# NthPortal/reservoir

Hardware: AMD Instinct MI355X
Metric: elements sampled/sec (Gelem/s) + % HBM roofline, 1B Long keys k=1024, 1/2/4/8 GPU (higher is better)
Workload: dtype int64

## Files before the change

reservoir_amd/csrc/rsv_device.h:

```cpp
#pragma once
#include <hip/hip_runtime.h>
#include <stdint.h>

namespace rsv {

struct u32x4 {
    uint32_t x, y, z, w;
};

constexpr uint32_t kPhiloxM0 = 0xD2511F53u;
constexpr uint32_t kPhiloxM1 = 0xCD9E8D57u;
constexpr uint32_t kPhiloxW0 = 0x9E3779B9u;
constexpr uint32_t kPhiloxW1 = 0xBB67AE85u;
constexpr uint32_t kDomainLevel1 = 0x80000000u;

__device__ __forceinline__ uint32_t xor3_key(uint32_t a, uint32_t b, uint32_t key) {
    return __builtin_amdgcn_bitop3_b32(a, b, key, 0x96);
}

__device__ __forceinline__ u32x4 philox4x32_10(uint32_t c0, uint32_t c1, uint32_t c2, uint32_t c3,
                                               uint32_t k0, uint32_t k1) {
#pragma unroll
    for (int r = 0; r < 10; ++r) {
        const uint64_t p0 = (uint64_t)kPhiloxM0 * c0;
        const uint64_t p1 = (uint64_t)kPhiloxM1 * c2;
        const uint32_t n0 = xor3_key((uint32_t)(p1 >> 32), c1, k0 + (uint32_t)r * kPhiloxW0);
        const uint32_t n2 = xor3_key((uint32_t)(p0 >> 32), c3, k1 + (uint32_t)r * kPhiloxW1);
        c0 = n0;
        c1 = (uint32_t)p1;
        c2 = n2;
        c3 = (uint32_t)p0;
    }
    return {c0, c1, c2, c3};
}

__device__ __forceinline__ u32x4 philox4x32_10_uniform_hi(uint32_t c0, uint32_t c1, uint32_t c2, uint32_t c3,
                                                          uint32_t k0, uint32_t k1, uint64_t add0 = 0) {
    const uint64_t p1u = (uint64_t)kPhiloxM1 * c2;
    const uint32_t n0u = (uint32_t)(p1u >> 32) ^ c1 ^ k0;
    const uint64_t p0 = (uint64_t)kPhiloxM0 * c0 + add0;
    uint32_t d2 = (uint32_t)(p0 >> 32) ^ (c3 ^ k1);
    const uint32_t d1u = (uint32_t)p1u;
    uint32_t d3 = (uint32_t)p0;
    const uint64_t q0u = (uint64_t)kPhiloxM0 * n0u;
    const uint64_t q1 = (uint64_t)kPhiloxM1 * d2;
    uint32_t c0v = (uint32_t)(q1 >> 32) ^ (d1u ^ (k0 + kPhiloxW0));
    uint32_t c2v = d3 ^ ((uint32_t)(q0u >> 32) ^ (k1 + kPhiloxW1));
    uint32_t c1v = (uint32_t)q1;
    uint32_t c3v = (uint32_t)q0u;
    {
        const uint64_t p0r = (uint64_t)kPhiloxM0 * c0v;
        const uint64_t p1r = (uint64_t)kPhiloxM1 * c2v;
        const uint32_t n0 = xor3_key((uint32_t)(p1r >> 32), c1v, k0 + 2u * kPhiloxW0);
        const uint32_t n2 = (uint32_t)(p0r >> 32) ^ (c3v ^ (k1 + 2u * kPhiloxW1));
        c0v = n0;
        c1v = (uint32_t)p1r;
        c2v = n2;
        c3v = (uint32_t)p0r;
    }
#pragma unroll
    for (int r = 3; r < 10; ++r) {
        const uint64_t p0r = (uint64_t)kPhiloxM0 * c0v;
        const uint64_t p1r = (uint64_t)kPhiloxM1 * c2v;
        const uint32_t n0 = xor3_key((uint32_t)(p1r >> 32), c1v, k0 + (uint32_t)r * kPhiloxW0);
        const uint32_t n2 = xor3_key((uint32_t)(p0r >> 32), c3v, k1 + (uint32_t)r * kPhiloxW1);
        c0v = n0;
        c1v = (uint32_t)p1r;
        c2v = n2;
        c3v = (uint32_t)p0r;
    }
    return {c0v, c1v, c2v, c3v};
}

__device__ __forceinline__ void philox4x32_10_uniform_hi_x2(uint32_t c0, uint32_t c1, uint32_t c2, uint32_t c3,
                                                            uint32_t k0, uint32_t k1, u32x4& a, u32x4& b) {
    const uint64_t p1u = (uint64_t)kPhiloxM1 * c2;
    const uint32_t n0u = (uint32_t)(p1u >> 32) ^ c1 ^ k0;
    const uint64_t pa = (uint64_t)kPhiloxM0 * c0;
    const uint64_t pb = (uint64_t)kPhiloxM0 * c0 + (uint64_t)kPhiloxM0 * 64u;
    const uint32_t da2 = xor3_key((uint32_t)(pa >> 32), c3, k1), db2 = xor3_key((uint32_t)(pb >> 32), c3, k1);
    const uint32_t d1u = (uint32_t)p1u;
    const uint32_t da3 = (uint32_t)pa, db3 = (uint32_t)pb;
    const uint64_t q0u = (uint64_t)kPhiloxM0 * n0u;
    const uint64_t qa = (uint64_t)kPhiloxM1 * da2, qb = (uint64_t)kPhiloxM1 * db2;
    uint32_t a0 = (uint32_t)(qa >> 32) ^ (d1u ^ (k0 + kPhiloxW0)), b0 = (uint32_t)(qb >> 32) ^ (d1u ^ (k0 + kPhiloxW0));
    uint32_t a2 = da3 ^ ((uint32_t)(q0u >> 32) ^ (k1 + kPhiloxW1)), b2 = db3 ^ ((uint32_t)(q0u >> 32) ^ (k1 + kPhiloxW1));
    uint32_t a1 = (uint32_t)qa, b1 = (uint32_t)qb;
    uint32_t a3 = (uint32_t)q0u, b3 = (uint32_t)q0u;
#pragma unroll
    for (int r = 2; r < 10; ++r) {
        const uint64_t pa0 = (uint64_t)kPhiloxM0 * a0, pb0 = (uint64_t)kPhiloxM0 * b0;
        const uint64_t pa1 = (uint64_t)kPhiloxM1 * a2, pb1 = (uint64_t)kPhiloxM1 * b2;
        const uint32_t na0 = xor3_key((uint32_t)(pa1 >> 32), a1, k0 + (uint32_t)r * kPhiloxW0);
        const uint32_t nb0 = xor3_key((uint32_t)(pb1 >> 32), b1, k0 + (uint32_t)r * kPhiloxW0);
        const uint32_t na2 = xor3_key((uint32_t)(pa0 >> 32), a3, k1 + (uint32_t)r * kPhiloxW1);
        const uint32_t nb2 = xor3_key((uint32_t)(pb0 >> 32), b3, k1 + (uint32_t)r * kPhiloxW1);
        a0 = na0;
        b0 = nb0;
        a1 = (uint32_t)pa1;
        b1 = (uint32_t)pb1;
        a2 = na2;
        b2 = nb2;
        a3 = (uint32_t)pa0;
        b3 = (uint32_t)pb0;
    }
    a = {a0, a1, a2, a3};
    b = {b0, b1, b2, b3};
}

constexpr uint32_t kPhiloxM0Inv = 0x991A7CDBu;
static_assert((uint32_t)(kPhiloxM0 * kPhiloxM0Inv) == 1u, "M0 inverse");

__device__ __forceinline__ void philox4x32_10_uniform_hi_x2_at(uint32_t gl, uint32_t m0v, uint64_t offa,
                                                               uint32_t c1, uint32_t c2, uint32_t c3,
                                                               uint32_t k0, uint32_t k1, u32x4& a, u32x4& b,
                                                               uint32_t& lo_a) {
    const uint64_t p1u = (uint64_t)kPhiloxM1 * c2;
    const uint32_t n0u = (uint32_t)(p1u >> 32) ^ c1 ^ k0;
    const uint64_t pa = (uint64_t)m0v * gl + offa;
    const uint64_t pb = (uint64_t)m0v * gl + (offa + (uint64_t)kPhiloxM0 * 64u);
    lo_a = (uint32_t)pa;
    const uint32_t c3k = c3 ^ k1;
    const uint32_t da2 = (uint32_t)(pa >> 32) ^ c3k, db2 = (uint32_t)(pb >> 32) ^ c3k;
    const uint32_t d1u = (uint32_t)p1u;
    const uint32_t da3 = (uint32_t)pa, db3 = (uint32_t)pb;
    const uint64_t q0u = (uint64_t)kPhiloxM0 * n0u;
    const uint64_t qa = (uint64_t)kPhiloxM1 * da2, qb = (uint64_t)kPhiloxM1 * db2;
    uint32_t a0 = (uint32_t)(qa >> 32) ^ (d1u ^ (k0 + kPhiloxW0)), b0 = (uint32_t)(qb >> 32) ^ (d1u ^ (k0 + kPhiloxW0));
    uint32_t a2 = da3 ^ ((uint32_t)(q0u >> 32) ^ (k1 + kPhiloxW1)), b2 = db3 ^ ((uint32_t)(q0u >> 32) ^ (k1 + kPhiloxW1));
    uint32_t a1 = (uint32_t)qa, b1 = (uint32_t)qb;
    uint32_t a3 = (uint32_t)q0u, b3 = (uint32_t)q0u;
    {
        const uint64_t pa0 = (uint64_t)kPhiloxM0 * a0, pb0 = (uint64_t)kPhiloxM0 * b0;
        const uint64_t pa1 = (uint64_t)kPhiloxM1 * a2, pb1 = (uint64_t)kPhiloxM1 * b2;
        const uint32_t na0 = xor3_key((uint32_t)(pa1 >> 32), a1, k0 + 2u * kPhiloxW0);
        const uint32_t nb0 = xor3_key((uint32_t)(pb1 >> 32), b1, k0 + 2u * kPhiloxW0);
        const uint32_t s3 = (uint32_t)q0u ^ (k1 + 2u * kPhiloxW1);
        const uint32_t na2 = (uint32_t)(pa0 >> 32) ^ s3, nb2 = (uint32_t)(pb0 >> 32) ^ s3;
        a0 = na0;
        b0 = nb0;
        a1 = (uint32_t)pa1;
        b1 = (uint32_t)pb1;
        a2 = na2;
        b2 = nb2;
        a3 = (uint32_t)pa0;
        b3 = (uint32_t)pb0;
    }
#pragma unroll
    for (int r = 3; r < 10; ++r) {
        const uint64_t pa0 = (uint64_t)kPhiloxM0 * a0, pb0 = (uint64_t)kPhiloxM0 * b0;
        const uint64_t pa1 = (uint64_t)kPhiloxM1 * a2, pb1 = (uint64_t)kPhiloxM1 * b2;
        const uint32_t na0 = xor3_key((uint32_t)(pa1 >> 32), a1, k0 + (uint32_t)r * kPhiloxW0);
        const uint32_t nb0 = xor3_key((uint32_t)(pb1 >> 32), b1, k0 + (uint32_t)r * kPhiloxW0);
        const uint32_t na2 = xor3_key((uint32_t)(pa0 >> 32), a3, k1 + (uint32_t)r * kPhiloxW1);
        const uint32_t nb2 = xor3_key((uint32_t)(pb0 >> 32), b3, k1 + (uint32_t)r * kPhiloxW1);
        a0 = na0;
        b0 = nb0;
        a1 = (uint32_t)pa1;
        b1 = (uint32_t)pb1;
        a2 = na2;
        b2 = nb2;
        a3 = (uint32_t)pa0;
        b3 = (uint32_t)pb0;
    }
    a = {a0, a1, a2, a3};
    b = {b0, b1, b2, b3};
}

struct DrawKey {
    uint32_t k0, k1;
    uint32_t s0, s1;
};

__device__ __forceinline__ u32x4 level0(const DrawKey& dk, uint64_t g0) {
    return philox4x32_10((uint32_t)g0, (uint32_t)(g0 >> 32), dk.s0, dk.s1, dk.k0, dk.k1);
}

__device__ __forceinline__ uint32_t word_of(const u32x4& w, uint32_t q) {
    return q == 0 ? w.x : q == 1 ? w.y : q == 2 ? w.z : w.w;
}

__device__ __forceinline__ uint32_t level0_byte(const u32x4& w, uint32_t e) {
    const uint32_t u = ((w.x >> e) & 0x10001u) | (((w.y >> e) & 0x10001u) << 2) |
                       (((w.z >> e) & 0x10001u) << 4) | (((w.w >> e) & 0x10001u) << 6);
    return (u & 0x55u) | ((u >> 15) & 0xAAu);
}

__device__ __forceinline__ uint64_t exact_j(const DrawKey& dk, uint64_t i, uint32_t b) {
    const uint64_t g1 = i >> 1;
    const u32x4 w =
        philox4x32_10((uint32_t)g1, (uint32_t)(g1 >> 32) | kDomainLevel1, dk.s0, dk.s1, dk.k0, dk.k1);
    const uint64_t L = (i & 1) ? (((uint64_t)w.z << 32) | w.w) : (((uint64_t)w.x << 32) | w.y);
    const uint64_t U = ((uint64_t)b << 56) | (L >> 8);
    return __umul64hi(U, i + 1);
}

__device__ __forceinline__ uint32_t planes_or(const u32x4& w) {
    const uint32_t x = w.x | w.y | w.z | w.w;
    return x | __builtin_amdgcn_alignbit(x, x, 16);
}

__device__ __forceinline__ uint32_t zero_byte_mask16(const u32x4& w) { return ~planes_or(w) & 0xFFFFu; }

__device__ __forceinline__ bool any_zero_byte(const u32x4& w) { return planes_or(w) != 0xFFFFFFFFu; }

__device__ __forceinline__ uint32_t lt_mask16(const u32x4& w, uint32_t T) {
    if (T >= 256u) return 0xFFFFu;
    uint32_t lt = 0, eq = 0xFFFFu;
#pragma unroll
    for (int p = 7; p >= 0; --p) {
        const uint32_t plane = (word_of(w, (uint32_t)p >> 1) >> (16 * (p & 1))) & 0xFFFFu;
        const uint32_t tm = 0u - ((T >> p) & 1u);
        lt |= eq & ~plane & tm;
        eq &= ~(plane ^ tm);
    }
    return lt & 0xFFFFu;
}

__host__ __device__ __forceinline__ uint64_t bswap64(uint64_t v) { return __builtin_bswap64(v); }

__host__ __device__ __forceinline__ int64_t byteswap64(int64_t v) {
    uint64_t hc = (uint64_t)v * 0x9e3779b97f4a7c15ULL;
    hc = bswap64(hc);
    return (int64_t)(hc * 0x9e3779b97f4a7c15ULL);
}

__host__ __device__ __forceinline__ int64_t scramble(int64_t r0, int64_t r1, int64_t hashed) {
    return byteswap64(r1 ^ byteswap64(r0 ^ hashed));
}

enum HashKind : int { kHashIdentity = 1, kHashJavaLong = 2, kHashJavaInt = 3, kHashPrecomputed = 4, kHashUuid = 5 };

__host__ __device__ __forceinline__ int64_t uuid_hash_code(uint64_t msb, uint64_t lsb) {
    const uint64_t hilo = msb ^ lsb;
    return (int64_t)(int32_t)((uint32_t)(hilo >> 32) ^ (uint32_t)hilo);
}

enum WideSrc : int { kWideSrcHashes = 0, kWideSrcUuid = 1 };

template <typename KeyT, int HASH>
__host__ __device__ __forceinline__ int64_t hash_of(KeyT key) {
    if constexpr (HASH == kHashJavaLong) {
        const uint64_t v = (uint64_t)(int64_t)key;
        return (int64_t)(int32_t)(uint32_t)(v ^ (v >> 32));
    } else if constexpr (HASH == kHashJavaInt) {
        return (int64_t)(int32_t)key;
    } else {
        return (int64_t)key;
    }
}

__device__ __forceinline__ uint32_t xor_lane32(uint32_t v, int s) {
    switch (s) {
    case 1: return (uint32_t)__builtin_amdgcn_mov_dpp((int)v, 0xB1, 0xF, 0xF, false);
    case 2: return (uint32_t)__builtin_amdgcn_mov_dpp((int)v, 0x4E, 0xF, 0xF, false);
    case 4: {
        const uint32_t up = (uint32_t)__builtin_amdgcn_mov_dpp((int)v, 0x104, 0xF, 0xF, false);
        const uint32_t dn = (uint32_t)__builtin_amdgcn_mov_dpp((int)v, 0x114, 0xF, 0xF, false);
        return (threadIdx.x & 4) ? dn : up;
    }
    case 8: return (uint32_t)__builtin_amdgcn_mov_dpp((int)v, 0x128, 0xF, 0xF, false);
    case 16: {
        const auto r = __builtin_amdgcn_permlane16_swap(v, v, false, false);
        return (threadIdx.x & 16) ? r[0] : r[1];
    }
    case 32: {
        const auto r = __builtin_amdgcn_permlane32_swap(v, v, false, false);
        return (threadIdx.x & 32) ? r[0] : r[1];
    }
    default: return (uint32_t)__shfl_xor((int)v, s);
    }
}

template <typename T>
__device__ __forceinline__ T xor_any(T v, int s) {
    if constexpr (sizeof(T) == 8) {
        const uint64_t x = (uint64_t)v;
        const uint32_t lo = xor_lane32((uint32_t)x, s), hi = xor_lane32((uint32_t)(x >> 32), s);
        return (T)(((uint64_t)hi << 32) | lo);
    } else {
        return (T)xor_lane32((uint32_t)v, s);
    }
}

__device__ __forceinline__ unsigned long long lanemask_lt64() {
    const uint32_t lane = threadIdx.x & 63;
    return lane ? (~0ull >> (64 - lane)) : 0ull;
}

__device__ __forceinline__ void publish_flag(uint32_t* flag, uint32_t gen) {
    asm volatile("s_waitcnt vmcnt(0)" ::: "memory");
    __syncthreads();
    if (threadIdx.x == 0) {
        __threadfence_system();
        __hip_atomic_store(flag, gen, __ATOMIC_RELEASE, __HIP_MEMORY_SCOPE_SYSTEM);
    }
}

}
```

reservoir_amd/csrc/rsv_elements.hip:

```cpp
#include <algorithm>

#include "rsv_device.h"
#include "rsv_internal.h"
#include "rsv_scan.h"

namespace rsv {

namespace {

constexpr int kBlock = 256;

constexpr int kK1Unroll = 2;

constexpr unsigned kK1Grid = 256 * 20;

constexpr int kK1Win = 12;
struct K1Lds {
    uint64_t q[kBlock / 64][k1q_cap<kK1Win>()];
    uint64_t cq[kBlock / 64][kQueue];
};

__device__ __forceinline__ bool k1_fast(uint64_t lo, uint64_t hi) {
    return (lo >> 33) == ((hi - 1) >> 33) && hi <= (1ull << 40);
}

struct K1Sched {
    uint32_t W1, A, B;
};

__global__ __launch_bounds__(kBlock) void k1_last_writer(DrawKey dk, uint32_t k, uint64_t lo,
                                                         uint64_t hi, uint64_t g_begin,
                                                         uint64_t n_groups,
                                                         unsigned long long* __restrict__ win, K1Sched sch) {
    __shared__ K1Lds L;
    const int w = threadIdx.x >> 6;
    if (k1_fast(lo, hi))
        k1_body_q<kK1Win, true>(dk, k, lo, hi, g_begin, n_groups, win, L.q[w], L.cq[w], sch.W1, sch.A, sch.B);
    else
        k1_body_q<kK1Win, false>(dk, k, lo, hi, g_begin, n_groups, win, L.q[w], L.cq[w], sch.W1, sch.A, sch.B);
}

template <typename Take, typename Empty, typename Keep>
__device__ __forceinline__ void slot_rule(int64_t j, unsigned long long wi, int64_t base, int64_t n, int fresh,
                                          Take&& take, Empty&& empty, Keep&& keep) {
    if (wi) take((int64_t)wi - base, (int64_t)wi, true);
    else if (j >= base && j < base + n) take(j - base, j, false);
    else if (fresh) empty((int64_t)-1);
    else keep();
}

template <typename KeyT, int R, bool kAgentWin>
__device__ __forceinline__ void resolve_registers_first(const KeyT* __restrict__ keys, int64_t base, int64_t n,
                                                        uint32_t k, unsigned long long* __restrict__ win,
                                                        KeyT* __restrict__ slot_key, int64_t* __restrict__ slot_idx,
                                                        int fresh, int64_t m, KeyT* dst, uint32_t* flag, uint32_t gen) {
    unsigned long long wi[R];
    KeyT v[R];
#pragma unroll
    for (int r = 0; r < R; ++r) {
        const uint32_t j = threadIdx.x + r * kBlock;
        if (j >= k) wi[r] = 0ull;
        else if (kAgentWin) wi[r] = __hip_atomic_load(&win[j], __ATOMIC_RELAXED, __HIP_MEMORY_SCOPE_AGENT);
        else wi[r] = win[j];
    }
#pragma unroll
    for (int r = 0; r < R; ++r) {
        const int64_t j = threadIdx.x + r * kBlock;
        if (j >= k) continue;
        KeyT x;
        slot_rule(
            j, wi[r], base, n, fresh, [&](int64_t off, int64_t, bool) { x = keys[off]; }, [&](int64_t) { x = 0; },
            [&] { x = slot_key[j]; });
        v[r] = x;
    }
#pragma unroll
    for (int r = 0; r < R; ++r) {
        const int64_t j = threadIdx.x + r * kBlock;
        if (j >= k) continue;
        const KeyT x = v[r];
        slot_rule(
            j, wi[r], base, n, fresh,
            [=](int64_t, int64_t idx, bool winner) {
                slot_key[j] = x;
                slot_idx[j] = idx;
                if (winner) win[j] = 0;
            },
            [=](int64_t idx) {
                slot_key[j] = 0;
                slot_idx[j] = idx;
            },
            [] {});
        if (j < m) dst[j] = x;
    }
    publish_flag(flag, gen);
}

constexpr uint32_t kK1FusedMaxK = 8 * kBlock;

template <typename KeyT>
__global__ __launch_bounds__(kBlock) void k1_resolve_publish(DrawKey dk, uint32_t k, uint64_t lo, uint64_t hi,
                                                             uint64_t g_begin, uint64_t n_groups,
                                                             unsigned long long* __restrict__ win,
                                                             uint32_t* ticket, const KeyT* __restrict__ keys,
                                                             int64_t base, int64_t n, KeyT* __restrict__ slot_key,
                                                             int64_t* __restrict__ slot_idx, int fresh, int64_t m,
                                                             KeyT* dst, uint32_t* flag, uint32_t gen, K1Sched sch) {
    __shared__ K1Lds L;
    __shared__ uint32_t last;
    const int w = threadIdx.x >> 6;
    if (k1_fast(lo, hi))
        k1_body_q<kK1Win, true>(dk, k, lo, hi, g_begin, n_groups, win, L.q[w], L.cq[w], sch.W1, sch.A, sch.B);
    else
        k1_body_q<kK1Win, false>(dk, k, lo, hi, g_begin, n_groups, win, L.q[w], L.cq[w], sch.W1, sch.A, sch.B);
    asm volatile("s_waitcnt vmcnt(0)" ::: "memory");
    __syncthreads();
    if (threadIdx.x == 0) {
        const uint32_t prev = __hip_atomic_fetch_add(ticket, 1u, __ATOMIC_RELAXED, __HIP_MEMORY_SCOPE_AGENT);
        last = prev == gridDim.x - 1;
        if (last) __hip_atomic_store(ticket, 0u, __ATOMIC_RELAXED, __HIP_MEMORY_SCOPE_AGENT);
    }
    __syncthreads();
    if (!last) return;
    __builtin_amdgcn_fence(__ATOMIC_ACQUIRE, "agent");
    resolve_registers_first<KeyT, kK1FusedMaxK / kBlock, true>(keys, base, n, k, win, slot_key, slot_idx, fresh, m, dst,
                                                               flag, gen);
}

template <typename KeyT, bool kPublish>
__global__ __launch_bounds__(kPublish ? 1024 : kBlock) void resolve_kernel(const KeyT* __restrict__ keys, int64_t base,
                                                                         int64_t n, uint32_t k,
                                                                         unsigned long long* __restrict__ win,
                                                                         KeyT* __restrict__ slot_key,
                                                                         int64_t* __restrict__ slot_idx, int fresh,
                                                                         int64_t m, KeyT* dst, uint32_t* flag,
                                                                         uint32_t gen) {
    const uint32_t stride = gridDim.x * blockDim.x;
    for (uint32_t j = blockIdx.x * blockDim.x + threadIdx.x; j < k; j += stride) {
        KeyT v = 0;
        slot_rule(
            j, win[j], base, n, fresh,
            [&](int64_t off, int64_t idx, bool winner) {
                slot_key[j] = v = keys[off];
                if (kPublish || slot_idx) slot_idx[j] = idx;
                if (winner) win[j] = 0;
            },
            [=](int64_t idx) {
                slot_key[j] = 0;
                if (kPublish || slot_idx) slot_idx[j] = idx;
            },
            [&] {
                if (kPublish) v = slot_key[j];
            });
        if (kPublish && (int64_t)j < m) dst[j] = v;
    }
    if (kPublish) publish_flag(flag, gen);
}

template <typename KeyT, int R>
__global__ __launch_bounds__(kBlock) void resolve_publish_small_kernel(const KeyT* __restrict__ keys, int64_t base,
                                                                       int64_t n, uint32_t k,
                                                                       unsigned long long* __restrict__ win,
                                                                       KeyT* __restrict__ slot_key,
                                                                       int64_t* __restrict__ slot_idx, int fresh,
                                                                       int64_t m, KeyT* dst, uint32_t* flag, uint32_t gen) {
    resolve_registers_first<KeyT, R, false>(keys, base, n, k, win, slot_key, slot_idx, fresh, m, dst, flag, gen);
}

__global__ __launch_bounds__(kBlock) void replay_kernel(const int64_t* __restrict__ ev_pos,
                                                        const int32_t* __restrict__ ev_slot,
                                                        int64_t n_events, uint32_t k,
                                                        unsigned long long* __restrict__ win) {
    const int64_t e = (int64_t)blockIdx.x * blockDim.x + threadIdx.x;
    if (e >= n_events) return;
    const int32_t s = ev_slot[e];
    const int64_t p = ev_pos[e];
    if (s >= 0 && (uint32_t)s < k && p >= 2) atomicMax(&win[s], (unsigned long long)(p - 1));
}

__global__ __launch_bounds__(kBlock) void export_draws_kernel(DrawKey dk, uint64_t i0, int64_t n,
                                                              uint64_t* __restrict__ out) {
    const int64_t t = (int64_t)blockIdx.x * blockDim.x + threadIdx.x;
    if (t >= n) return;
    const uint64_t i = i0 + (uint64_t)t;
    const u32x4 w = level0(dk, i >> 4);
    out[t] = exact_j(dk, i, level0_byte(w, (uint32_t)(i & 15)));
}

template <typename KeyT>
struct StridedParts {
    using Key = KeyT;
    const int64_t* idx;
    const KeyT* key;
    int64_t part_len;
    __device__ int64_t index(int32_t p, uint32_t j) const { return idx[(int64_t)p * part_len + j]; }
    __device__ void take(int32_t p, uint32_t j, KeyT* slot_key) const { slot_key[j] = key[(int64_t)p * part_len + j]; }
};

template <typename KeyT>
struct PackedRows {
    using Key = KeyT;
    const int64_t* rows;
    int64_t stride;
    uint32_t k;
    __device__ int64_t index(int32_t p, uint32_t j) const { return rows[(int64_t)p * stride + j]; }
    __device__ void take(int32_t p, uint32_t j, KeyT* slot_key) const {
        slot_key[j] = (KeyT)rows[(int64_t)p * stride + k + j];
    }
};

struct StridedWideParts {
    using Key = uint32_t;
    const int64_t* idx;
    const uint32_t* key;
    int64_t part_len;
    uint32_t words;
    __device__ int64_t index(int32_t p, uint32_t j) const { return idx[(int64_t)p * part_len + j]; }
    __device__ void take(int32_t p, uint32_t j, uint32_t* slot_key) const {
        const uint32_t* src = key + ((size_t)p * part_len + j) * words;
        for (uint32_t q = 0; q < words; ++q) slot_key[(size_t)j * words + q] = src[q];
    }
};

struct PackedWideRows {
    using Key = uint32_t;
    const int64_t* rows;
    int64_t stride;
    uint32_t k, words;
    __device__ int64_t index(int32_t p, uint32_t j) const { return rows[(int64_t)p * stride + j]; }
    __device__ void take(int32_t p, uint32_t j, uint32_t* slot_key) const {
        const uint32_t* src = (const uint32_t*)(rows + (int64_t)p * stride + k) + (size_t)j * words;
        for (uint32_t q = 0; q < words; ++q) slot_key[(size_t)j * words + q] = src[q];
    }
};

template <typename Src>
__device__ __forceinline__ int32_t merge_winner(const Src& src, int32_t parts, uint32_t j, int64_t& best) {
    int32_t from = -1;
    for (int32_t p = 0; p < parts; ++p) {
        const int64_t idx = src.index(p, j);
        if (idx > best) {
            best = idx;
            from = p;
        }
    }
    return from;
}

template <typename Src, bool kPublish>
__global__ __launch_bounds__(kPublish ? 1024 : kBlock) void merge_kernel(Src src, int32_t parts, uint32_t k,
                                                                       int64_t* __restrict__ slot_idx,
                                                                       typename Src::Key* __restrict__ slot_key,
                                                                       int64_t m, typename Src::Key* dst,
                                                                       uint32_t* flag, uint32_t gen) {
    const uint32_t stride = gridDim.x * blockDim.x;
    for (uint32_t j = blockIdx.x * blockDim.x + threadIdx.x; j < k; j += stride) {
        int64_t best = slot_idx[j];
        const int32_t from = merge_winner(src, parts, j, best);
        if (from >= 0) {
            slot_idx[j] = best;
            src.take(from, j, slot_key);
        }
        if (kPublish && (int64_t)j < m) dst[j] = slot_key[j];
    }
    if (kPublish) publish_flag(flag, gen);
}

template <typename KeyT>
__global__ __launch_bounds__(kBlock) void export_packed_kernel(const int64_t* __restrict__ slot_idx,
                                                               const KeyT* __restrict__ slot_key, uint32_t k,
                                                               int64_t* __restrict__ row) {
    const uint32_t j = blockIdx.x * blockDim.x + threadIdx.x;
    if (j >= k) return;
    row[j] = slot_idx[j];
    row[k + j] = (int64_t)slot_key[j];
}

__global__ __launch_bounds__(1024) void resolve_wide_kernel(const uint32_t* __restrict__ keys, int64_t base,
                                                            int64_t n, uint32_t k, uint32_t words,
                                                            unsigned long long* __restrict__ win,
                                                            uint32_t* __restrict__ slot_key,
                                                            int64_t* __restrict__ slot_idx, int fresh, int64_t m,
                                                            uint32_t* dst, uint32_t* flag, uint32_t gen) {
    const uint32_t stride = gridDim.x * blockDim.x;
    for (uint32_t j = blockIdx.x * blockDim.x + threadIdx.x; j < k; j += stride) {
        const uint32_t* src = nullptr;
        bool write = true;
        slot_rule(
            j, win[j], base, n, fresh,
            [&](int64_t off, int64_t idx, bool winner) {
                src = keys + (size_t)off * words;
                slot_idx[j] = idx;
                if (winner) win[j] = 0;
            },
            [=](int64_t idx) { slot_idx[j] = idx; }, [&] { write = false; });
        uint32_t* o = slot_key + (size_t)j * words;
        const bool out = dst && (int64_t)j < m;
        for (uint32_t q = 0; q < words; ++q) {
            const uint32_t v = src ? src[q] : (write ? 0u : o[q]);
            if (write) o[q] = v;
            if (out) dst[(size_t)j * words + q] = v;
        }
    }
    if (dst) publish_flag(flag, gen);
}

__global__ __launch_bounds__(kBlock) void export_packed_wide_kernel(const int64_t* __restrict__ slot_idx,
                                                                    const uint32_t* __restrict__ slot_key, uint32_t k,
                                                                    uint32_t words, int64_t* __restrict__ row) {
    const uint32_t j = blockIdx.x * blockDim.x + threadIdx.x;
    if (j >= k) return;
    row[j] = slot_idx[j];
    uint32_t* o = (uint32_t*)(row + k) + (size_t)j * words;
    for (uint32_t q = 0; q < words; ++q) o[q] = slot_key[(size_t)j * words + q];
}

inline DrawKey make_key(const DrawParams& dp) {
    return DrawKey{(uint32_t)dp.seed, (uint32_t)(dp.seed >> 32), (uint32_t)dp.stream,
                   (uint32_t)(dp.stream >> 32)};
}

inline unsigned grid_for(uint64_t items, unsigned cap = ~0u) {
// ... 353 lines not shown
```

reservoir_amd/csrc/rsv_scan.h:

```cpp
#pragma once
#include <algorithm>

#include "rsv_device.h"

namespace rsv {

constexpr uint32_t kQueue = 128;
constexpr uint64_t kIndexMask = (1ull << 56) - 1;

__device__ __forceinline__ uint32_t clip_mask16(uint64_t i0, uint64_t lo, uint64_t hi) {
    uint32_t m = 0xFFFFu;
    if (i0 < lo) m = (lo - i0 >= 16) ? 0u : ((0xFFFFu << (uint32_t)(lo - i0)) & 0xFFFFu);
    if (i0 + 16 > hi) m &= (hi <= i0) ? 0u : (0xFFFFu >> (uint32_t)(16 - (hi - i0)));
    return m;
}

__device__ __forceinline__ uint32_t candidate_mask16(const u32x4& w, uint64_t i0, uint64_t dense_lim) {
    if (i0 + 1 >= dense_lim) return zero_byte_mask16(w);
    const float Tf = __fdividef((float)dense_lim, (float)(i0 + 1));
    if (Tf > 300.0f) return 0xFFFFu;
    uint32_t T = (uint32_t)Tf;
    if ((uint64_t)T * (i0 + 1) < dense_lim) ++T;
    if (T > 0 && (uint64_t)(T - 1) * (i0 + 1) >= dense_lim) --T;
    return lt_mask16(w, T > 256u ? 256u : T);
}

template <class Hit>
__device__ __forceinline__ void resolve_entry(const DrawKey& dk, uint64_t e, uint32_t k, Hit& hit) {
    const uint64_t i = e & kIndexMask;
    const uint64_t j = exact_j(dk, i, (uint32_t)(e >> 56));
    if (j < k) hit((uint32_t)j, i);
}

template <class Hit>
__device__ __forceinline__ void enqueue_block(const DrawKey& dk, const u32x4& w, uint64_t i0,
                                              uint32_t mask, uint64_t* q, uint32_t& qn,
                                              uint32_t lane, uint32_t k, Hit& hit) {
    while (__any(mask != 0)) {
        const bool has = mask != 0;
        const unsigned long long bal = __ballot(has);
        if (has) {
            const uint32_t e = __builtin_ctz(mask);
            mask &= mask - 1;
            q[qn + __popcll(bal & lanemask_lt64())] = ((uint64_t)level0_byte(w, e) << 56) | (i0 + e);
        }
        qn += (uint32_t)__popcll(bal);
        if (qn >= 64) {
            qn -= 64;
            __builtin_amdgcn_wave_barrier();
            resolve_entry(dk, q[qn + lane], k, hit);
            __builtin_amdgcn_wave_barrier();
        }
    }
}

template <class Hit>
__device__ __forceinline__ void drain_queue(const DrawKey& dk, const uint64_t* q, uint32_t& qn,
                                            uint32_t lane, uint32_t k, Hit& hit) {
    __builtin_amdgcn_wave_barrier();
    if (lane < qn) resolve_entry(dk, q[lane], k, hit);
    qn = 0;
    __builtin_amdgcn_wave_barrier();
}


template <class Hit>
__device__ __forceinline__ void resolve_block(const DrawKey& dk, bool valid, uint64_t g, uint64_t lo,
                                              uint64_t hi, uint64_t dense_lim, uint32_t k, uint64_t* cq,
                                              uint32_t& cqn, uint32_t lane, Hit& hit) {
    const u32x4 w = level0(dk, g);
    const uint64_t i0 = g << 4;
    uint32_t mask = valid ? candidate_mask16(w, i0, dense_lim) : 0u;
    if (i0 < lo || i0 + 16 > hi) mask &= clip_mask16(i0, lo, hi);
    if (mask) {
        const uint32_t e = __builtin_ctz(mask);
        mask &= mask - 1;
        const uint64_t j = exact_j(dk, i0 + e, level0_byte(w, e));
        if (j < k) hit((uint32_t)j, i0 + e);
    }
    enqueue_block(dk, w, i0, mask, cq, cqn, lane, k, hit);
}

__device__ __forceinline__ uint32_t fold16(const u32x4& w) {
    const uint32_t x = w.x | w.y | w.z | w.w;
    uint32_t y;
    asm("v_or_b32_sdwa %0, %1, %1 dst_sel:WORD_0 dst_unused:UNUSED_PAD src0_sel:WORD_0 src1_sel:WORD_1\n\t"
        "s_nop 0"
        : "=v"(y)
        : "v"(x));
    return y;
}

__device__ __forceinline__ u32x4 level1_b0_words(const DrawKey& dk, uint64_t i, bool hi_uniform, uint32_t c1u) {
    const uint64_t g1 = i >> 1;
    if (hi_uniform) return philox4x32_10_uniform_hi((uint32_t)g1, c1u, dk.s0, dk.s1, dk.k0, dk.k1);
    return philox4x32_10((uint32_t)g1, (uint32_t)(g1 >> 32) | kDomainLevel1, dk.s0, dk.s1, dk.k0, dk.k1);
}

__device__ __forceinline__ uint32_t fold_pair(const u32x4& a, const u32x4& b) {
    const uint32_t xa = a.x | a.y | a.z | a.w, xb = b.x | b.y | b.z | b.w;
    uint32_t z;
    asm("v_or_b32_sdwa %0, %1, %1 dst_sel:WORD_0 dst_unused:UNUSED_PAD src0_sel:WORD_0 src1_sel:WORD_1\n\t"
        "s_nop 0\n\t"
        "v_or_b32_sdwa %0, %2, %2 dst_sel:WORD_1 dst_unused:UNUSED_PRESERVE src0_sel:WORD_0 src1_sel:WORD_1\n\t"
        "s_nop 0"
        : "=&v"(z)
        : "v"(xa), "v"(xb));
    return z;
}

template <int W>
constexpr uint32_t k1q_cap() { return 64u * (1u + W / 2); }
constexpr uint32_t kQueueWaves = 4;

template <int W = 12, bool FAST = false>
__device__ __forceinline__ void k1_body_q(const DrawKey& dk, uint32_t k, uint64_t lo, uint64_t hi, uint64_t g_begin,
                                          uint64_t n_groups, unsigned long long* __restrict__ win, uint64_t* q,
                                          uint64_t* cq, uint32_t W1 = 0, uint32_t A = 0, uint32_t B = 0,
                                          uint32_t* pool = nullptr) {
    static_assert(W % 2 == 0, "half windows");
    constexpr int U = 2;
    const uint32_t lane = threadIdx.x & 63;
    uint32_t qn = 0, cqn = 0;
    auto hit = [&](uint32_t j, uint64_t i) { atomicMax(&win[j], (unsigned long long)i); };
    const uint64_t dense_lim = 256ull * k;
    const uint32_t ng = (uint32_t)n_groups;
    const uint64_t g_sparse = (dense_lim + 14) >> 4;
    const uint32_t off_sparse = g_sparse <= g_begin ? 0u : (uint32_t)std::min<uint64_t>(g_sparse - g_begin, ng);
    const uint32_t stride = gridDim.x * blockDim.x * U;
    const uint32_t c1u = (uint32_t)__builtin_amdgcn_readfirstlane((int)((uint32_t)(lo >> 33) | kDomainLevel1));
    const bool hi_uniform = (lo >> 33) == ((hi - 1) >> 33);
    const bool pre_ok = hi <= (1ull << 40);
    const uint64_t k_hi = (uint64_t)k << 32, k_24 = (uint64_t)k << 24;
    int32_t dpend = 0;
    const uint32_t g0 = (uint32_t)g_begin;
    uint32_t base = __builtin_amdgcn_readfirstlane((blockIdx.x * blockDim.x + (threadIdx.x & ~63u)) * U);
    const uint32_t ghi = (uint32_t)__builtin_amdgcn_readfirstlane((int)(uint32_t)(g_begin >> 32));
    uint32_t gl = g0 + base + lane;
    const uint32_t off_steady =
        __builtin_amdgcn_readfirstlane((int)std::max<uint32_t>(off_sparse, (lo & 15) ? 1u : 0u));
    const uint32_t ng_steady = __builtin_amdgcn_readfirstlane((int)(ng - ((hi & 15) ? 1u : 0u)));

    auto resolve = [&](bool valid, uint64_t ent) {
        const uint32_t gt = (uint32_t)ent * kPhiloxM0Inv, off = gt - g0, z = (uint32_t)(ent >> 32);
        __builtin_assume(!valid || z != 0xFFFFFFFFu);
        bool dense = false;
        if (dpend > 0) {
            dense = valid && ((z & 0xFFFFu) == 0 || (z >> 16) == 0);
            const unsigned long long db = __builtin_amdgcn_ballot_w64(dense);
            if (db) {
                resolve_block(dk, dense, g_begin + off, lo, hi, dense_lim, k, cq, cqn, lane, hit);
                resolve_block(dk, dense && off + 64 < ng, g_begin + off + 64, lo, hi, dense_lim, k, cq, cqn, lane, hit);
                dpend -= std::min<int32_t>(dpend, (int32_t)__popcll(db));
            }
        }
        const uint32_t zm = (valid && !dense) ? ~z : 0u;
        uint32_t rest = 0;
        if (zm) {
            const uint32_t e = __builtin_ctz(zm);
            rest = zm & (zm - 1);
            if constexpr (FAST) {
                const uint32_t bl = gt + ((e & 16u) << 2);
                const uint32_t g1lo = (bl << 3) | ((e & 15u) >> 1);
                const u32x4 w = philox4x32_10_uniform_hi(g1lo, c1u, dk.s0, dk.s1, dk.k0, dk.k1);
                const bool odd = e & 1u;
                const uint32_t Lh = odd ? w.z : w.x;
                const uint32_t i8 = (ghi << 28) | (bl >> 4);
                if ((uint64_t)(Lh >> 8) * i8 < k_24) {
                    const uint64_t i = ((((uint64_t)ghi << 32) | bl) << 4) | (e & 15u);
                    const uint64_t L = ((uint64_t)Lh << 32) | (odd ? w.w : w.y);
                    const uint64_t j = __umul64hi(L >> 8, i + 1);
                    if (j < k) hit((uint32_t)j, i);
                }
            } else {
                const uint64_t i = ((g_begin + off + ((e >> 4) << 6)) << 4) + (e & 15u);
                const u32x4 w = level1_b0_words(dk, i, hi_uniform, c1u);
                const uint32_t Lh = (i & 1) ? w.z : w.x;
                const bool maybe = !pre_ok || (uint64_t)(Lh >> 8) * (i + 1) < k_hi;
                if (maybe) {
                    const uint64_t L = ((uint64_t)Lh << 32) | ((i & 1) ? w.w : w.y);
                    const uint64_t j = __umul64hi(L >> 8, i + 1);
                    if (j < k) hit((uint32_t)j, i);
                }
            }
        }
        const unsigned long long bal = __builtin_amdgcn_ballot_w64(rest != 0);
        if (bal) {
            if (rest) {
                const uint32_t pos = __builtin_amdgcn_mbcnt_hi((uint32_t)(bal >> 32), __builtin_amdgcn_mbcnt_lo((uint32_t)bal, 0u));
                q[qn + pos] = (uint64_t)(uint32_t)ent | ((uint64_t)~rest << 32);
            }
            qn += (uint32_t)__popcll(bal);
        }
    };
    auto rounds = [&]() {
        while (qn >= 64) {
            qn -= 64;
            __builtin_amdgcn_wave_barrier();
            const uint64_t ent = q[qn + lane];
            __builtin_amdgcn_wave_barrier();
            resolve(true, ent);
            __builtin_amdgcn_wave_barrier();
        }
    };
    auto append = [&](bool has, uint32_t gt, uint32_t z) {
        const unsigned long long bal = __builtin_amdgcn_ballot_w64(has);
        if (has) {
            const uint32_t pos = __builtin_amdgcn_mbcnt_hi((uint32_t)(bal >> 32), __builtin_amdgcn_mbcnt_lo((uint32_t)bal, 0u));
            q[qn + pos] = (uint64_t)gt | ((uint64_t)z << 32);
        }
        qn += (uint32_t)__popcll(bal);
    };

    const uint32_t q_s = (uint32_t)__builtin_amdgcn_readfirstlane((int)(uint32_t)(uintptr_t)q);
    uint32_t m0v;
    asm volatile("v_mov_b32 %0, %1" : "=v"(m0v) : "s"(kPhiloxM0));
    auto steady = [&](uint32_t d) {
        u32x4 w0, w1;
        uint32_t glo;
        philox4x32_10_uniform_hi_x2_at(gl, m0v, (uint64_t)kPhiloxM0 * d, ghi, dk.s0, dk.s1, dk.k0, dk.k1, w0, w1, glo);
        const uint32_t xa = w0.x | w0.y | w0.z | w0.w, xb = w1.x | w1.y | w1.z | w1.w;
        uint32_t z;
        unsigned long long m;
        asm("v_or_b32_sdwa %0, %2, %2 dst_sel:WORD_0 dst_unused:UNUSED_PAD src0_sel:WORD_0 src1_sel:WORD_1\n\t"
            "s_nop 0\n\t"
            "v_or_b32_sdwa %0, %3, %3 dst_sel:WORD_1 dst_unused:UNUSED_PRESERVE src0_sel:WORD_0 src1_sel:WORD_1\n\t"
            "s_nop 0\n\t"
            "v_cmp_ne_u32_e64 %1, -1, %0"
            : "=&v"(z), "=s"(m)
            : "v"(xa), "v"(xb));
        const uint32_t pos = __builtin_amdgcn_mbcnt_hi((uint32_t)(m >> 32), __builtin_amdgcn_mbcnt_lo((uint32_t)m, 0u));
        const uint32_t sb = q_s + 8u * qn;
        const uint64_t ent = (uint64_t)glo | ((uint64_t)z << 32);
        unsigned long long sv;
        uint32_t addr;
        asm volatile("v_lshl_add_u32 %1, %2, 3, %3\n\t"
                     "s_mov_b64 %0, exec\n\t"
                     "s_mov_b64 exec, %4\n\t"
                     "ds_write_b64 %1, %5\n\t"
                     "s_mov_b64 exec, %0"
                     : "=&s"(sv), "=&v"(addr)
                     : "v"(pos), "s"(sb), "s"(m), "v"(ent)
                     : "memory");
        qn += (uint32_t)__popcll(m);
    };
    auto partial = [&](uint32_t b) {
        u32x4 w[U];
#pragma unroll
        for (int u = 0; u < U; ++u)
            w[u] = philox4x32_10_uniform_hi(gl, ghi, dk.s0, dk.s1, dk.k0, dk.k1, (uint64_t)kPhiloxM0 * (64u * u));
        uint32_t z;
        bool has;
        if (b >= off_steady && b + U * 64 <= ng_steady) {
            z = fold_pair(w[0], w[1]);
            has = z != 0xFFFFFFFFu;
        } else {
            uint32_t y[U];
            bool hb[U];
#pragma unroll
            for (int u = 0; u < U; ++u) {
                const uint32_t off = b + u * 64 + lane;
                const uint64_t i0 = (g_begin + off) << 4;
                const bool dense = i0 + 1 < dense_lim;
                y[u] = off >= ng ? 0xFFFFu
                                 : dense ? 0u : (fold16(w[u]) | (~clip_mask16(i0, lo, hi) & 0xFFFFu));
                hb[u] = (off < ng) & (dense | ((uint16_t)y[u] != 0xFFFFu));
            }
            z = (y[0] & 0xFFFFu) | (y[1] << 16);
            has = hb[0] | hb[1];
        }
        dpend += (int32_t)__popcll(__builtin_amdgcn_ballot_w64(has && ((z & 0xFFFFu) == 0 || (z >> 16) == 0)));
        append(has, gl * kPhiloxM0, z);
        __builtin_amdgcn_wave_barrier();
        rounds();
    };
    if (A > 0) {
        constexpr uint32_t UB = (W / 2) * U * 64;
        const uint32_t units = (ng + UB - 1) / UB;
        const uint32_t wg = __builtin_amdgcn_readfirstlane((blockIdx.x * blockDim.x + threadIdx.x) >> 6);
        const uint32_t nB = gridDim.x * (blockDim.x >> 6) - W1;
        const bool ga = wg < W1;
        const uint32_t cnt = ga ? A : B, u_step = ga ? W1 : nB, u_first = ga ? wg : W1 * A + (wg - W1);
        for (uint32_t j = 0; j < cnt; ++j) {
            const uint32_t u = u_first + j * u_step;
            if (u >= units) break;
            uint32_t ub = u * UB;
            gl = g0 + ub + lane;
            if (ub >= off_steady && ub + UB <= ng_steady) {
#pragma unroll
                for (int t = 0; t < W / 2; ++t) steady(t * (U * 64));
                __builtin_amdgcn_wave_barrier();
                rounds();
            } else {
                for (int t = 0; t < W / 2 && ub < ng; ++t, ub += U * 64, gl += U * 64) partial(ub);
            }
        }
        base = ng;
    }
    while (base < ng) {
        if (base >= off_steady && (uint64_t)base + (uint64_t)(W - 1) * stride + U * 64 <= ng_steady) {
#pragma unroll
            for (int h = 0; h < 2; ++h) {
#pragma unroll
                for (int t = 0; t < W / 2; ++t) steady(t * stride);
                gl += (W / 2) * stride;
                __builtin_amdgcn_wave_barrier();
                rounds();
            }
            base += W * stride;
        } else {
            for (int t = 0; t < W && base < ng; ++t, base += stride, gl += stride) {
                partial(base);
            }
        }
    }
    if (pool) {
        constexpr uint32_t cap = k1q_cap<W>(), NW = kQueueWaves;
        const uint32_t wv = threadIdx.x >> 6;
        const uint64_t* q0 = q - (size_t)wv * cap;
        for (;;) {
            if (lane == 0) pool[wv] = qn | (dpend > 0 ? 0x80000000u : 0u);
            __syncthreads();
            uint32_t c[NW], T = 0, anyd = 0;
#pragma unroll
            for (uint32_t v = 0; v < NW; ++v) {
                const uint32_t pv = (uint32_t)__builtin_amdgcn_readfirstlane((int)pool[v]);
                c[v] = pv & 0x7FFFFFFFu;
                anyd |= pv >> 31;
                T += c[v];
            }
            if (T == 0) break;
            uint32_t o = 64u * wv + lane, src = 0;
            const bool valid = o < T;
#pragma unroll
            for (uint32_t v = 0; v + 1 < NW; ++v)
                if (src == v && o >= c[v]) {
                    o -= c[v];
                    src = v + 1;
                }
            const uint64_t ent = valid ? q0[(size_t)src * cap + o] : 0ull;
            __syncthreads();
            qn = 0;
            dpend = anyd ? (1 << 30) : 0;
            if (64u * wv < T) resolve(valid, ent);
        }
    } else {
        while (qn > 0) {
            __builtin_amdgcn_wave_barrier();
            const uint32_t nv = std::min<uint32_t>(qn, 64u);
            qn -= nv;
            const bool valid = lane < nv;
            const uint64_t ent = valid ? q[qn + lane] : 0ull;
            __builtin_amdgcn_wave_barrier();
            resolve(valid, ent);
        }
    }
    __builtin_amdgcn_wave_barrier();
    drain_queue(dk, cq, cqn, lane, k, hit);
}

}
```

Measured before the change: 11490.

## Queue candidates as 4-block quads with 64-bit masks in LDS scan kernel

The level-1 scan now produces one queue entry per four 64-group blocks instead of two. Each entry is a 16-byte LDS struct holding two 32-bit zero masks plus the group id, and pointers are advanced with v_lshl_add_u64 instead of recomputing multiplies. The intent is to halve queue append and resolve traffic and to shrink per-window bookkeeping. In exchange each resolve pass handles wider masks and does more dense-block ballots. The block-wide pooled queue draining path is removed, so draining falls back to per-wave only.

```diff
diff --git a/reservoir_amd/csrc/rsv_device.h b/reservoir_amd/csrc/rsv_device.h
--- a/reservoir_amd/csrc/rsv_device.h
+++ b/reservoir_amd/csrc/rsv_device.h
@@ -111,15 +111,11 @@
 constexpr uint32_t kPhiloxM0Inv = 0x991A7CDBu;
 static_assert((uint32_t)(kPhiloxM0 * kPhiloxM0Inv) == 1u, "M0 inverse");
 
-__device__ __forceinline__ void philox4x32_10_uniform_hi_x2_at(uint32_t gl, uint32_t m0v, uint64_t offa,
-                                                               uint32_t c1, uint32_t c2, uint32_t c3,
-                                                               uint32_t k0, uint32_t k1, u32x4& a, u32x4& b,
-                                                               uint32_t& lo_a) {
+__device__ __forceinline__ void philox4x32_10_uniform_hi_x2_p(uint64_t pa, uint64_t pb, uint32_t c1, uint32_t c2,
+                                                              uint32_t c3, uint32_t k0, uint32_t k1, u32x4& a,
+                                                              u32x4& b) {
     const uint64_t p1u = (uint64_t)kPhiloxM1 * c2;
     const uint32_t n0u = (uint32_t)(p1u >> 32) ^ c1 ^ k0;
-    const uint64_t pa = (uint64_t)m0v * gl + offa;
-    const uint64_t pb = (uint64_t)m0v * gl + (offa + (uint64_t)kPhiloxM0 * 64u);
-    lo_a = (uint32_t)pa;
     const uint32_t c3k = c3 ^ k1;
     const uint32_t da2 = (uint32_t)(pa >> 32) ^ c3k, db2 = (uint32_t)(pb >> 32) ^ c3k;
     const uint32_t d1u = (uint32_t)p1u;
@@ -167,6 +163,16 @@
     b = {b0, b1, b2, b3};
 }
 
+__device__ __forceinline__ void philox4x32_10_uniform_hi_x2_at(uint32_t gl, uint32_t m0v, uint64_t offa,
+                                                               uint32_t c1, uint32_t c2, uint32_t c3,
+                                                               uint32_t k0, uint32_t k1, u32x4& a, u32x4& b,
+                                                               uint32_t& lo_a) {
+    const uint64_t pa = (uint64_t)m0v * gl + offa;
+    const uint64_t pb = (uint64_t)m0v * gl + (offa + (uint64_t)kPhiloxM0 * 64u);
+    lo_a = (uint32_t)pa;
+    philox4x32_10_uniform_hi_x2_p(pa, pb, c1, c2, c3, k0, k1, a, b);
+}
+
 struct DrawKey {
     uint32_t k0, k1;
     uint32_t s0, s1;
diff --git a/reservoir_amd/csrc/rsv_elements.hip b/reservoir_amd/csrc/rsv_elements.hip
--- a/reservoir_amd/csrc/rsv_elements.hip
+++ b/reservoir_amd/csrc/rsv_elements.hip
@@ -16,7 +16,7 @@
 
 constexpr int kK1Win = 12;
 struct K1Lds {
-    uint64_t q[kBlock / 64][k1q_cap<kK1Win>()];
+    K1Quad q[kBlock / 64][k1q_cap<kK1Win>()];
     uint64_t cq[kBlock / 64][kQueue];
 };
 
diff --git a/reservoir_amd/csrc/rsv_scan.h b/reservoir_amd/csrc/rsv_scan.h
--- a/reservoir_amd/csrc/rsv_scan.h
+++ b/reservoir_amd/csrc/rsv_scan.h
@@ -109,17 +109,28 @@
     return z;
 }
 
+__device__ __forceinline__ unsigned long long quad_mark(uint32_t z0, uint32_t z1, uint64_t& z) {
+    z = (uint64_t)z0 | ((uint64_t)z1 << 32);
+    unsigned long long m;
+    asm("v_cmp_ne_u64_e64 %0, -1, %1" : "=s"(m) : "v"(z));
+    return m;
+}
+
+struct alignas(16) K1Quad {
+    uint32_t z0, z1;
+    uint32_t glo;
+    uint32_t pad;
+};
 template <int W>
-constexpr uint32_t k1q_cap() { return 64u * (1u + W / 2); }
-constexpr uint32_t kQueueWaves = 4;
+constexpr uint32_t k1q_cap() { return 64u * (1u + W / 4); }
 
 template <int W = 12, bool FAST = false>
 __device__ __forceinline__ void k1_body_q(const DrawKey& dk, uint32_t k, uint64_t lo, uint64_t hi, uint64_t g_begin,
-                                          uint64_t n_groups, unsigned long long* __restrict__ win, uint64_t* q,
-                                          uint64_t* cq, uint32_t W1 = 0, uint32_t A = 0, uint32_t B = 0,
-                                          uint32_t* pool = nullptr) {
-    static_assert(W % 2 == 0, "half windows");
+                                          uint64_t n_groups, unsigned long long* __restrict__ win, K1Quad* q,
+                                          uint64_t* cq, uint32_t W1 = 0, uint32_t A = 0, uint32_t B = 0) {
+    static_assert(W % 4 == 0, "half windows of whole quads");
     constexpr int U = 2;
+    constexpr uint32_t QB = 4 * 64;
     const uint32_t lane = threadIdx.x & 63;
     uint32_t qn = 0, cqn = 0;
     auto hit = [&](uint32_t j, uint64_t i) { atomicMax(&win[j], (unsigned long long)i); };
@@ -127,40 +138,52 @@
     const uint32_t ng = (uint32_t)n_groups;
     const uint64_t g_sparse = (dense_lim + 14) >> 4;
     const uint32_t off_sparse = g_sparse <= g_begin ? 0u : (uint32_t)std::min<uint64_t>(g_sparse - g_begin, ng);
-    const uint32_t stride = gridDim.x * blockDim.x * U;
+    const uint32_t stride = gridDim.x * blockDim.x * 4;
     const uint32_t c1u = (uint32_t)__builtin_amdgcn_readfirstlane((int)((uint32_t)(lo >> 33) | kDomainLevel1));
     const bool hi_uniform = (lo >> 33) == ((hi - 1) >> 33);
     const bool pre_ok = hi <= (1ull << 40);
     const uint64_t k_hi = (uint64_t)k << 32, k_24 = (uint64_t)k << 24;
     int32_t dpend = 0;
     const uint32_t g0 = (uint32_t)g_begin;
-    uint32_t base = __builtin_amdgcn_readfirstlane((blockIdx.x * blockDim.x + (threadIdx.x & ~63u)) * U);
+    uint32_t base = __builtin_amdgcn_readfirstlane((blockIdx.x * blockDim.x + (threadIdx.x & ~63u)) * 4);
     const uint32_t ghi = (uint32_t)__builtin_amdgcn_readfirstlane((int)(uint32_t)(g_begin >> 32));
-    uint32_t gl = g0 + base + lane;
+    const uint32_t gl0 = g0 + lane;
     const uint32_t off_steady =
         __builtin_amdgcn_readfirstlane((int)std::max<uint32_t>(off_sparse, (lo & 15) ? 1u : 0u));
     const uint32_t ng_steady = __builtin_amdgcn_readfirstlane((int)(ng - ((hi & 15) ? 1u : 0u)));
 
-    auto resolve = [&](bool valid, uint64_t ent) {
-        const uint32_t gt = (uint32_t)ent * kPhiloxM0Inv, off = gt - g0, z = (uint32_t)(ent >> 32);
-        __builtin_assume(!valid || z != 0xFFFFFFFFu);
-        bool dense = false;
+    auto resolve = [&](bool valid, const K1Quad& ent) {
+        const uint32_t gt = ent.glo * kPhiloxM0Inv, off = gt - g0;
+        uint64_t z = valid ? ((uint64_t)ent.z0 | ((uint64_t)ent.z1 << 32)) : ~0ull;
+        __builtin_assume(!valid || z != ~0ull);
+        bool any = valid;
         if (dpend > 0) {
-            dense = valid && ((z & 0xFFFFu) == 0 || (z >> 16) == 0);
-            const unsigned long long db = __builtin_amdgcn_ballot_w64(dense);
-            if (db) {
-                resolve_block(dk, dense, g_begin + off, lo, hi, dense_lim, k, cq, cqn, lane, hit);
-                resolve_block(dk, dense && off + 64 < ng, g_begin + off + 64, lo, hi, dense_lim, k, cq, cqn, lane, hit);
-                dpend -= std::min<int32_t>(dpend, (int32_t)__popcll(db));
-            }
-        }
-        const uint32_t zm = (valid && !dense) ? ~z : 0u;
-        uint32_t rest = 0;
-        if (zm) {
-            const uint32_t e = __builtin_ctz(zm);
-            rest = zm & (zm - 1);
+            const uint32_t z0 = (uint32_t)z, z1 = (uint32_t)(z >> 32);
+            const bool d0 = (z0 & 0xFFFFu) == 0 || (z0 >> 16) == 0, d1 = (z1 & 0xFFFFu) == 0 || (z1 >> 16) == 0;
+            const unsigned long long db0 = __builtin_amdgcn_ballot_w64(d0), db1 = __builtin_amdgcn_ballot_w64(d1);
+            if (db0) {
+                resolve_block(dk, d0, g_begin + off, lo, hi, dense_lim, k, cq, cqn, lane, hit);
+                resolve_block(dk, d0 && off + 64 < ng, g_begin + off + 64, lo, hi, dense_lim, k, cq, cqn, lane, hit);
+            }
+            if (db1) {
+                resolve_block(dk, d1 && off + 128 < ng, g_begin + off + 128, lo, hi, dense_lim, k, cq, cqn, lane, hit);
+                resolve_block(dk, d1 && off + 192 < ng, g_begin + off + 192, lo, hi, dense_lim, k, cq, cqn, lane, hit);
+            }
+            if (db0 | db1) dpend -= std::min<int32_t>(dpend, (int32_t)__popcll(db0 | db1));
+            if (d0) z |= 0xFFFFFFFFull;
+            if (d1) z |= 0xFFFFFFFF00000000ull;
+            any = z != ~0ull;
+        }
+        uint64_t rest = ~0ull;
+        if (any) {
+            const uint64_t t = z + 1;
+            uint32_t f0, f1;
+            asm("v_ffbl_b32 %0, %1" : "=v"(f0) : "v"((uint32_t)t));
+            asm("v_ffbl_b32 %0, %1" : "=v"(f1) : "v"((uint32_t)(t >> 32)));
+            const uint32_t e = std::min<uint32_t>(f0, f1 | 32u);
+            rest = z | t;
             if constexpr (FAST) {
-                const uint32_t bl = gt + ((e & 16u) << 2);
+                const uint32_t bl = gt + (__builtin_amdgcn_ubfe(e, 4u, 2u) << 6);
                 const uint32_t g1lo = (bl << 3) | ((e & 15u) >> 1);
                 const u32x4 w = philox4x32_10_uniform_hi(g1lo, c1u, dk.s0, dk.s1, dk.k0, dk.k1);
                 const bool odd = e & 1u;
@@ -184,11 +207,15 @@
                 }
             }
         }
-        const unsigned long long bal = __builtin_amdgcn_ballot_w64(rest != 0);
+        const bool more = rest != ~0ull;
+        const unsigned long long bal = __builtin_amdgcn_ballot_w64(more);
         if (bal) {
-            if (rest) {
+            if (more) {
                 const uint32_t pos = __builtin_amdgcn_mbcnt_hi((uint32_t)(bal >> 32), __builtin_amdgcn_mbcnt_lo((uint32_t)bal, 0u));
-                q[qn + pos] = (uint64_t)(uint32_t)ent | ((uint64_t)~rest << 32);
+                K1Quad& o = q[qn + pos];
+                o.z0 = (uint32_t)rest;
+                o.z1 = (uint32_t)(rest >> 32);
+                o.glo = ent.glo;
             }
             qn += (uint32_t)__popcll(bal);
         }
@@ -197,7 +224,7 @@
         while (qn >= 64) {
             qn -= 64;
             __builtin_amdgcn_wave_barrier();
-            const uint64_t ent = q[qn + lane];
+            const K1Quad ent = q[qn + lane];
             __builtin_amdgcn_wave_barrier();
             resolve(true, ent);
             __builtin_amdgcn_wave_barrier();
@@ -207,7 +234,10 @@
         const unsigned long long bal = __builtin_amdgcn_ballot_w64(has);
         if (has) {
             const uint32_t pos = __builtin_amdgcn_mbcnt_hi((uint32_t)(bal >> 32), __builtin_amdgcn_mbcnt_lo((uint32_t)bal, 0u));
-            q[qn + pos] = (uint64_t)gt | ((uint64_t)z << 32);
+            K1Quad& o = q[qn + pos];
+            o.z0 = z;
+            o.z1 = 0xFFFFFFFFu;
+            o.glo = gt;
         }
         qn += (uint32_t)__popcll(bal);
     };
@@ -215,40 +245,54 @@
     const uint32_t q_s = (uint32_t)__builtin_amdgcn_readfirstlane((int)(uint32_t)(uintptr_t)q);
     uint32_t m0v;
     asm volatile("v_mov_b32 %0, %1" : "=v"(m0v) : "s"(kPhiloxM0));
-    auto steady = [&](uint32_t d) {
-        u32x4 w0, w1;
-        uint32_t glo;
-        philox4x32_10_uniform_hi_x2_at(gl, m0v, (uint64_t)kPhiloxM0 * d, ghi, dk.s0, dk.s1, dk.k0, dk.k1, w0, w1, glo);
-        const uint32_t xa = w0.x | w0.y | w0.z | w0.w, xb = w1.x | w1.y | w1.z | w1.w;
-        uint32_t z;
-        unsigned long long m;
-        asm("v_or_b32_sdwa %0, %2, %2 dst_sel:WORD_0 dst_unused:UNUSED_PAD src0_sel:WORD_0 src1_sel:WORD_1\n\t"
-            "s_nop 0\n\t"
-            "v_or_b32_sdwa %0, %3, %3 dst_sel:WORD_1 dst_unused:UNUSED_PRESERVE src0_sel:WORD_0 src1_sel:WORD_1\n\t"
-            "s_nop 0\n\t"
-            "v_cmp_ne_u32_e64 %1, -1, %0"
-            : "=&v"(z), "=s"(m)
-            : "v"(xa), "v"(xb));
+    auto step = [](uint64_t p, uint64_t c) {
+        uint64_t r;
+        asm("v_lshl_add_u64 %0, %1, 0, %2" : "=v"(r) : "v"(p), "s"(c));
+        return r;
+    };
+    const uint64_t c64 = (uint64_t)kPhiloxM0 * 64u;
+    auto steady = [&](uint64_t p) {
+        u32x4 w0, w1, w2, w3;
+        const uint32_t glo = (uint32_t)p;
+        const uint64_t pb = step(p, c64);
+        philox4x32_10_uniform_hi_x2_p(p, pb, ghi, dk.s0, dk.s1, dk.k0, dk.k1, w0, w1);
+        const uint32_t z0 = fold_pair(w0, w1);
+        const uint64_t pc = step(pb, c64), pd = step(pc, c64);
+        philox4x32_10_uniform_hi_x2_p(pc, pd, ghi, dk.s0, dk.s1, dk.k0, dk.k1, w2, w3);
+        const uint32_t z1 = fold_pair(w2, w3);
+        uint64_t z;
+        const unsigned long long m = quad_mark(z0, z1, z);
         const uint32_t pos = __builtin_amdgcn_mbcnt_hi((uint32_t)(m >> 32), __builtin_amdgcn_mbcnt_lo((uint32_t)m, 0u));
-        const uint32_t sb = q_s + 8u * qn;
-        const uint64_t ent = (uint64_t)glo | ((uint64_t)z << 32);
+        const uint32_t sb = q_s + 16u * qn;
         unsigned long long sv;
         uint32_t addr;
-        asm volatile("v_lshl_add_u32 %1, %2, 3, %3\n\t"
+        asm volatile("v_lshl_add_u32 %1, %2, 4, %3\n\t"
                      "s_mov_b64 %0, exec\n\t"
                      "s_mov_b64 exec, %4\n\t"
                      "ds_write_b64 %1, %5\n\t"
+                     "ds_write_b32 %1, %6 offset:8\n\t"
                      "s_mov_b64 exec, %0"
                      : "=&s"(sv), "=&v"(addr)
-                     : "v"(pos), "s"(sb), "s"(m), "v"(ent)
+                     : "v"(pos), "s"(sb), "s"(m), "v"(z), "v"(glo)
                      : "memory");
         qn += (uint32_t)__popcll(m);
-    };
-    auto partial = [&](uint32_t b) {
+        return pd;
+    };
+    auto half_window = [&](uint32_t b, uint64_t c_next) {
+        uint64_t p = (uint64_t)m0v * gl0 + (uint64_t)kPhiloxM0 * b;
+#pragma unroll
+        for (int t = 0; t < W / 4; ++t) {
+            const uint64_t pd = steady(p);
+            if (t + 1 < W / 4) p = step(pd, c_next);
+        }
+        __builtin_amdgcn_wave_barrier();
+        rounds();
+    };
+    auto partial = [&](uint32_t b, uint32_t gb) {
         u32x4 w[U];
 #pragma unroll
         for (int u = 0; u < U; ++u)
-            w[u] = philox4x32_10_uniform_hi(gl, ghi, dk.s0, dk.s1, dk.k0, dk.k1, (uint64_t)kPhiloxM0 * (64u * u));
+            w[u] = philox4x32_10_uniform_hi(gb, ghi, dk.s0, dk.s1, dk.k0, dk.k1, (uint64_t)kPhiloxM0 * (64u * u));
         uint32_t z;
         bool has;
         if (b >= off_steady && b + U * 64 <= ng_steady) {
@@ -270,12 +314,12 @@
             has = hb[0] | hb[1];
         }
         dpend += (int32_t)__popcll(__builtin_amdgcn_ballot_w64(has && ((z & 0xFFFFu) == 0 || (z >> 16) == 0)));
-        append(has, gl * kPhiloxM0, z);
+        append(has, gb * kPhiloxM0, z);
         __builtin_amdgcn_wave_barrier();
         rounds();
     };
     if (A > 0) {
-        constexpr uint32_t UB = (W / 2) * U * 64;
+        constexpr uint32_t UB = (W / 4) * QB;
         const uint32_t units = (ng + UB - 1) / UB;
         const uint32_t wg = __builtin_amdgcn_readfirstlane((blockIdx.x * blockDim.x + threadIdx.x) >> 6);
         const uint32_t nB = gridDim.x * (blockDim.x >> 6) - W1;
@@ -285,75 +329,36 @@
             const uint32_t u = u_first + j * u_step;
             if (u >= units) break;
             uint32_t ub = u * UB;
-            gl = g0 + ub + lane;
             if (ub >= off_steady && ub + UB <= ng_steady) {
+                half_window(ub, c64);
+            } else {
+                for (int t = 0; t < W / 2 && ub < ng; ++t, ub += U * 64) partial(ub, gl0 + ub);
+            }
+        }
+        base = ng;
+    }
+    const uint64_t c_stride = (uint64_t)kPhiloxM0 * (stride - 3 * 64u);
+    while (base < ng) {
+        if (base >= off_steady && (uint64_t)base + (uint64_t)(W / 2 - 1) * stride + QB <= ng_steady) {
 #pragma unroll
-                for (int t = 0; t < W / 2; ++t) steady(t * (U * 64));
-                __builtin_amdgcn_wave_barrier();
-                rounds();
-            } else {
-                for (int t = 0; t < W / 2 && ub < ng; ++t, ub += U * 64, gl += U * 64) partial(ub);
-            }
-        }
-        base = ng;
-    }
-    while (base < ng) {
-        if (base >= off_steady && (uint64_t)base + (uint64_t)(W - 1) * stride + U * 64 <= ng_steady) {
-#pragma unroll
-            for (int h = 0; h < 2; ++h) {
-#pragma unroll
-                for (int t = 0; t < W / 2; ++t) steady(t * stride);
-                gl += (W / 2) * stride;
-                __builtin_amdgcn_wave_barrier();
-                rounds();
-            }
-            base += W * stride;
+            for (int h = 0; h < 2; ++h) half_window(base + h * (W / 4) * stride, c_stride);
+            base += (W / 2) * stride;
         } else {
-            for (int t = 0; t < W && base < ng; ++t, base += stride, gl += stride) {
-                partial(base);
-            }
-        }
-    }
-    if (pool) {
-        constexpr uint32_t cap = k1q_cap<W>(), NW = kQueueWaves;
-        const uint32_t wv = threadIdx.x >> 6;
-        const uint64_t* q0 = q - (size_t)wv * cap;
-        for (;;) {
-            if (lane == 0) pool[wv] = qn | (dpend > 0 ? 0x80000000u : 0u);
-            __syncthreads();
-            uint32_t c[NW], T = 0, anyd = 0;
-#pragma unroll
-            for (uint32_t v = 0; v < NW; ++v) {
-                const uint32_t pv = (uint32_t)__builtin_amdgcn_readfirstlane((int)pool[v]);
-                c[v] = pv & 0x7FFFFFFFu;
-                anyd |= pv >> 31;
-                T += c[v];
-            }
-            if (T == 0) break;
-            uint32_t o = 64u * wv + lane, src = 0;
-            const bool valid = o < T;
-#pragma unroll
-            for (uint32_t v = 0; v + 1 < NW; ++v)
-                if (src == v && o >= c[v]) {
-                    o -= c[v];
-                    src = v + 1;
-                }
-            const uint64_t ent = valid ? q0[(size_t)src * cap + o] : 0ull;
-            __syncthreads();
-            qn = 0;
-            dpend = anyd ? (1 << 30) : 0;
-            if (64u * wv < T) resolve(valid, ent);
-        }
-    } else {
-        while (qn > 0) {
-            __builtin_amdgcn_wave_barrier();
-            const uint32_t nv = std::min<uint32_t>(qn, 64u);
-            qn -= nv;
-            const bool valid = lane < nv;
-            const uint64_t ent = valid ? q[qn + lane] : 0ull;
-            __builtin_amdgcn_wave_barrier();
-            resolve(valid, ent);
-        }
+            for (int t = 0; t < W / 2 && base < ng; ++t, base += stride) {
+                partial(base, gl0 + base);
+                if (base + U * 64 < ng) partial(base + U * 64, gl0 + base + U * 64);
+            }
+        }
+    }
+    while (qn > 0) {
+        __builtin_amdgcn_wave_barrier();
+        const uint32_t nv = std::min<uint32_t>(qn, 64u);
+        qn -= nv;
+        const bool valid = lane < nv;
+        K1Quad ent{0xFFFFFFFFu, 0xFFFFFFFFu, 0u, 0u};
+        if (valid) ent = q[qn + lane];
+        __builtin_amdgcn_wave_barrier();
+        resolve(valid, ent);
     }
     __builtin_amdgcn_wave_barrier();
     drain_queue(dk, cq, cqn, lane, k, hit);
```

Result: no change. 11560, median of 6 (+0.6%).
